# a-rtemis99/hpc_suffix_array

Measured on AMD Instinct MI355X. Metric: suffixes sorted/sec + ms/doubling-round, 1 GiB input at 1/2/4/8 MI355X, higher is better.
Workload: dtype u32

## Files before the change

### hpc_suffix_array_amd/_native.py

```python
from __future__ import annotations

import ctypes
import os
import subprocess

PKG_DIR = os.path.dirname(os.path.abspath(__file__))
LIB_PATH = os.path.join(PKG_DIR, "lib", "libsa_hip.so")
LIB_PATH = os.environ.get("SA_LIB_PATH", LIB_PATH)
CSRC = os.path.join(PKG_DIR, "csrc")

SA_MAX_ROUNDS = 64
KERNEL_KINDS = ["init", "hist_first", "hist_keys", "scan", "scatter_first", "scatter_keys",
                "heads", "heads_scan", "rerank", "seg_count", "seg_scan", "seg_write", "alphabet", "pack",
                "sort_u", "windows", "local_sort", "pivot_keys", "pivot_count", "pivot_write"]
SCHEDULE_PACKED = 0
SCHEDULE_REFERENCE = 1
ROUND1_AUTO = 0
ROUND1_LSD = 1
ROUND1_BUCKETED = 2
SA_K_COUNT = len(KERNEL_KINDS)
FIND_AUTO = 0
FIND_LANE = 1
FIND_WAVE = 2
FIND_LANE_MAX = 3584
# ... 17 lines not shown
               "sa_bwt_device", "sa_bwt", "sa_inverse_device", "sa_inverse",
               "sa_locate_device", "sa_locate",
               "sa_dist_begin", "sa_dist_cuts", "sa_dist_plan_cuts", "sa_dist_reserve", "sa_dist_release", "sa_dist_round1", "sa_dist_req_count", "sa_dist_req_fill",
               "sa_dist_answer", "sa_dist_refine",
               "sa_last_error", "sa_host_syncs", "sa_device_count", "sa_version", "sa_struct_size"]


class SAError(RuntimeError):
    """A libsa_hip entry point returned an error code."""


DEBUG_FLAGS = {"no_cmp": 0x1, "no_pk8": 0x2, "no_pad": 0x4, "pad_overflow": 0x8, "no_fast32": 0x10,
               "no_pivot": 0x20, "perm_always": 0x40, "no_xq": 0x80, "xq_overflow": 0x100,
               "no_tied": 0x200, "no_key1_round": 0x400, "no_eonly": 0x800,
               "eonly": 0x1000, "fast32_small": 0x2000, "no_round2_fused": 0x4000,
               "ls_one_wg": 0x8000}


def debug_bits(names) -> int:
    bits = 0
    for x in names or ():
        if x not in DEBUG_FLAGS:
            raise ValueError(f"unknown debug flag {x!r} (one of {sorted(DEBUG_FLAGS)})")
        bits |= DEBUG_FLAGS[x]
    return bits


class SaOpts(ctypes.Structure):
    _fields_ = [("profile", ctypes.c_int32), ("schedule", ctypes.c_int32), ("init_chars", ctypes.c_int32),
                ("radix", ctypes.c_int32), ("round1", ctypes.c_int32), ("debug", ctypes.c_uint32),
                ("span_extra", ctypes.c_int32), ("tune", ctypes.c_int32)]
# ... 13 lines not shown
        ("prefix_len", ctypes.c_uint64 * SA_MAX_ROUNDS),
        ("schedule", ctypes.c_int32),
        ("init_chars", ctypes.c_int32),
        ("sigma", ctypes.c_int32),
        ("sparse_ranks", ctypes.c_int32),
        ("round1", ctypes.c_int32),
        ("largest_window", ctypes.c_int32),
        ("model_bytes", ctypes.c_uint64),
        ("kern_ms", ctypes.c_double * SA_K_COUNT),
        ("kern_launches", ctypes.c_uint64 * SA_K_COUNT),
        ("kern_bytes", ctypes.c_uint64 * SA_K_COUNT),
        ("round1_segments", ctypes.c_int32),
        ("round1_layout", ctypes.c_int32),
        ("round_bytes", ctypes.c_uint64 * SA_MAX_ROUNDS),
        ("round1_windows", ctypes.c_int32 * 4),
    ]

    def to_dict(self) -> dict:
        r = self.rounds
        return {
            "rounds": r,
            "total_ms": self.total_ms,
            "h2d_ms": self.h2d_ms,
            "d2h_ms": self.d2h_ms,
            "round_ms": list(self.round_ms[:r]),
            "distinct": [int(x) for x in self.distinct[:r]],
            "passes": list(self.passes[:r]),
            "sorted_n": [int(x) for x in self.sorted_n[:r]],
            "prefix_len": [int(x) for x in self.prefix_len[:r]],
            "schedule": "reference" if self.schedule == SCHEDULE_REFERENCE else "packed",
            "init_chars": self.init_chars,
            "sigma": self.sigma,
            "sparse_ranks": bool(self.sparse_ranks),
            "round1": {ROUND1_LSD: "lsd", ROUND1_BUCKETED: "bucketed", 3: "pivot"}.get(self.round1, "lsd"),
            "largest_window": self.largest_window,
            "round1_segments": {0: "exact", 1: "padded", 2: "padded-overflow", 3: "striped-records",
                                4: "striped-records-overflow"}.get(self.round1_segments, "exact"),
            "round1_layout": {"compact": bool(self.round1_layout & 1), "pk8": bool(self.round1_layout & 2),
                              "xq": bool(self.round1_layout & 4), "eonly": bool(self.round1_layout & 8)},
            "reference_model_bytes": int(self.model_bytes),
            "round_bytes": [int(x) for x in self.round_bytes[:r]],
            "round1_windows": [int(x) for x in self.round1_windows],
            "kernels": {k: {"ms": self.kern_ms[i], "launches": int(self.kern_launches[i]),
                            "bytes": int(self.kern_bytes[i])} for i, k in enumerate(KERNEL_KINDS)},
        }


DIST_OK = 0
DIST_UNSUPPORTED = 1
DIST_UNBALANCED = 2


class SaDistInfo(ctypes.Structure):
    _fields_ = [("status", ctypes.c_int32), ("sigma", ctypes.c_int32), ("K", ctypes.c_int32),
                ("bucket_bits", ctypes.c_int32), ("m", ctypes.c_uint64), ("sa_off", ctypes.c_uint64),
                ("m_max", ctypes.c_uint64), ("bucket_lo", ctypes.c_uint32), ("bucket_hi", ctypes.c_uint32),
                ("round1_ok", ctypes.c_int32), ("reserved", ctypes.c_int32), ("heads", ctypes.c_uint64),
# ... 159 lines not shown
```

### hpc_suffix_array_amd/csrc/sa_build.hip

```cpp
#include <hip/hip_runtime.h>

#include <algorithm>
#include <atomic>
#include <chrono>
#include <cstdarg>
#include <cstdio>
#include <cstdlib>
#include <cstring>
#include <mutex>
#include <string>
#include <thread>
#include <vector>

#include "../../include/sa_hip.h"

#ifndef SA_ALPHA_GRID
#define SA_ALPHA_GRID 2048
#endif

#include "sa_bucket.h"
#include "sa_check.h"
#include "sa_kernels.h"
#include "sa_lcp.h"
#include "sa_limits.h"
// ... 119 lines not shown
    uint32_t* member = nullptr;
    uint32_t* hist = nullptr;
    uint32_t* totals = nullptr;
    uint32_t* counts = nullptr;
    uint32_t* words = nullptr;
    uint32_t* alpha = nullptr;
    uint16_t* code = nullptr;
    uint32_t* host_words = nullptr;
    hipEvent_t ev[sa::kEvPool + sa::kRoundEv + 1];
    int ev_ready = 0;
    sa::DistState* dist = nullptr;
    uint32_t dbg = 0;
    int32_t span_extra = 0;
    int32_t tune = 0;
    bool dna = false;
    bool samples_pending = false;
};

namespace sa {

static uint64_t pad_capacity(uint64_t n) { return n + n / 8 + (1ull << 22); }

static uint64_t pad_elems(uint64_t n) {
    const uint64_t m = align_up(std::max<uint64_t>(n, 1), 64);
    return (n >= (1ull << 26) && n <= (1ull << 31)) ? align_up(pad_capacity(n), 64) : m;
}

constexpr uint64_t kMaxRadix = 1024;
static uint64_t tile_states_bytes(uint64_t n) { return ((n + kTile - 1) / kTile + 1) * kMaxRadix * 8; }

// ... 1068 lines not shown
    *D = Dr + Dt;
    *m = mrr + T;
    *G = Gr + Gt;
    *P = 2 + Pr;
    return SA_OK;
}

static int build_packed(sa_context* c, const uint8_t* d_text, uint64_t n, uint32_t* d_sa, hipStream_t s,
                        const sa_opts* opts, sa_stats* st, Timer& tm) {
    int rc = SA_OK;
    rc = ensure_u_capacity(c, n);
    if (rc) return rc;
    tm.round_mark();
    uint32_t* h_alpha = c->host_words + 64;
    uint16_t* h_code = reinterpret_cast<uint16_t*>(c->host_words + 320);
    SA_HIP(hipMemsetAsync(c->alpha, 0, 8 * 4, s));
    tm.begin(SA_K_ALPHABET);
    {
        const uint32_t grid = (uint32_t)std::min<uint64_t>((n + kBlock * 16 - 1) / (kBlock * 16), SA_ALPHA_GRID);
        hipLaunchKernelGGL(k_alphabet, dim3(grid), dim3(kBlock), 0, s, d_text, n, c->alpha);
    }
    tm.end();
    SA_HIP(hipGetLastError());
    add_bytes(st, SA_K_ALPHABET, n);
    SA_HIP(hipMemcpyAsync(h_alpha, c->alpha, 8 * 4, hipMemcpyDeviceToHost, s));
    const uint32_t tail_n = (uint32_t)std::min<uint64_t>(n, (uint64_t)kMaxK);
    uint8_t* h_tail = reinterpret_cast<uint8_t*>(c->host_words + 2048);
    SA_HIP(hipMemcpyAsync(h_tail, d_text + (n - tail_n), tail_n, hipMemcpyDeviceToHost, s));
    SA_HIP(host_sync(s));
    uint32_t sigma = 0;
    for (int b = 0; b < 256; ++b) h_code[b] = ((h_alpha[b >> 5] >> (b & 31)) & 1u) ? (uint16_t)(++sigma) : 0;
    SA_HIP(hipMemcpyAsync(c->code, h_code, 256 * 2, hipMemcpyHostToDevice, s));
    c->dna = sigma == 4 && h_code['A'] && h_code['C'] && h_code['G'] && h_code['T'];
    uint32_t K = choose_chars(sigma, n, opts ? opts->init_chars : 0);
    const uint64_t base = (uint64_t)sigma + 1;
    const Chunking ch = plan_chunks(n);
    uint64_t* keys1 = nullptr;
    uint32_t ksh1 = 0;
    c->samples_pending = false;
    uint32_t P = 0;

    BucketPlan bp;
    const int r1 = opts ? opts->round1 : SA_ROUND1_AUTO;
    const uint32_t Kb = (opts && opts->init_chars > 0) || sigma <= 1 ? K : min_chars(sigma, n);
    bool bucketed = plan_bucketed(sigma, n, Kb, r1, c->radix, &bp, 1, (c->dbg & SA_DEBUG_NO_CMP) ? 0 : 1);
    if (bucketed && bp.bs.cmp && short_suffix_ties(h_tail, n, tail_n, h_code, sigma, bp.bs.s, bp.bs.R))
        bucketed = plan_bucketed(sigma, n, Kb, r1, c->radix, &bp, 1, 0);
    const bool force_eonly = (c->dbg & SA_DEBUG_EONLY) != 0;
    if (bucketed && bp.bs.cmp == 1 && ((sigma & (sigma - 1)) != 0 || force_eonly) && !(c->dbg & SA_DEBUG_NO_EONLY)) {
        const uint32_t hb = bp.bs.bb - kLoBits;
        BucketPlan b2;
        if ((force_eonly || !plan_pk8(bp, hb, c->dbg, true)) && plan_bucketed(sigma, n, Kb, r1, c->radix, &b2, 1, 2) &&
            (force_eonly || plan_pk8(b2, hb, c->dbg, true)) &&
            !short_suffix_ties(h_tail, n, tail_n, h_code, sigma, b2.bs.s, b2.bs.R, b2.K))
            bp = b2;
    }
    bool fused = false;
    bool r1_pivot = false;
    uint64_t D = 0, m = 0, G = 0;
    uint64_t seg1[3] = {0, 0, 0};
    int r2 = 0;
    if (bucketed) {
        bool done = false;
        rc = round1_bucketed(c, d_text, n, d_sa, bp, full_range(bp, n), s, tm, st, &done, &fused, seg1, &ksh1, true,
                             true, &r2);
        if (rc) return rc;
        bucketed = done;
        if (done) {
            keys1 = c->keys[0];
            P = 2;
            K = bp.K;
        }
    }
    if (!bucketed) {
        const uint32_t bits1 = key_bits(base, K);
        SA_TRACE("packed: sigma=%u K=%u bits=%u", sigma, K, bits1);
        uint64_t top = 1;
        for (uint32_t t = 1; t < K; ++t) top *= base;
        if (c->radix == 0) {
            rc = onesweep_prepare(c, s);
            if (rc) return rc;
        }
        tm.begin(SA_K_PACK);
        hipLaunchKernelGGL(k_pack_text, dim3(ch.chunks), dim3(kBlock), 0, s, d_text, n, (const uint16_t*)c->code, ch,
                           base, top, K, c->keys[1], c->hist, c->radix == 0 ? (bits1 + 7) / 8 : 0u, os_ghist(c));
        tm.end();
        SA_HIP(hipGetLastError());
        add_bytes(st, SA_K_PACK, 9 * n);
// ... 1258 lines not shown
```

### hpc_suffix_array_amd/csrc/sa_kernels.h

```cpp
#pragma once
#include <hip/hip_runtime.h>
#include <stdint.h>

#include "sa_search.h"

namespace sa {

constexpr int kWave = 64;
constexpr int kBlock = 256;
constexpr int kWaves = kBlock / kWave;
constexpr int kItems = 16;
constexpr int kTile = kBlock * kItems;
constexpr int kWaveTile = kWave * kItems;
constexpr int kRadix = 256;

__device__ __forceinline__ uint32_t lane_id() { return threadIdx.x & (kWave - 1); }
__device__ __forceinline__ uint32_t wave_id() { return threadIdx.x / kWave; }
__device__ __forceinline__ uint64_t lanemask_lt() { return (1ull << lane_id()) - 1ull; }

struct SrcRank {
    const uint32_t* __restrict__ rank;
    uint64_t n;
    uint64_t h;
    uint32_t w;
// ... 623 lines not shown
#pragma unroll
        for (int j = 0; j < kItems; ++j) {
            const uint64_t e = w0 + (uint64_t)j * kWave + lane_id();
            if (e < e1) {
                const uint32_t x = idx[e];
                if (x < ch.n) rank[x] = woff + (uint32_t)__popcll(m[j] & le_mask);
            }
            woff += (uint32_t)__popcll(m[j]);
        }
        run += ttot;
    }
    (void)s_tmp;
}


__global__ __launch_bounds__(kBlock) void k_alphabet(const uint8_t* __restrict__ text, uint64_t n,
                                                     uint32_t* __restrict__ present) {
    __shared__ uint32_t s_m[kBlock * 9];
    uint32_t* m = s_m + threadIdx.x * 9;
#pragma unroll
    for (int i = 0; i < 8; ++i) m[i] = 0;
    auto add = [&](uint32_t b) { atomicOr(&m[b >> 5], 1u << (b & 31u)); };
    const uint64_t stride = (uint64_t)gridDim.x * kBlock * 16;
    auto whole = [&](uint64_t i) { return i + 16 <= n && (((uintptr_t)(text + i)) & 15) == 0; };
    uint64_t i = ((uint64_t)blockIdx.x * kBlock + threadIdx.x) * 16;
    uint4 v = make_uint4(0u, 0u, 0u, 0u);
    if (i < n && whole(i)) v = *reinterpret_cast<const uint4*>(text + i);
    uint32_t step = 0;
    for (; i < n; i += stride) {
        if (step && (step & (step - 1)) == 0) {
// ... 24 lines not shown
                for (int q = 0; q < 4; ++q)
#pragma unroll
                    for (int b = 0; b < 4; ++b) bits |= 1u << ((w4[q] >> (8 * b)) & 31u);
                atomicOr(&m[(o & 0xFFu) >> 5], bits);
            } else {
#pragma unroll
                for (int q = 0; q < 4; ++q)
#pragma unroll
                    for (int b = 0; b < 4; ++b) add((w4[q] >> (8 * b)) & 0xFFu);
            }
        } else {
            for (uint64_t j = i; j < n && j < i + 16; ++j) add(text[j]);
        }
        v = vn;
    }
    __shared__ uint32_t s_or[8];
    if (threadIdx.x < 8) s_or[threadIdx.x] = 0;
    __syncthreads();
#pragma unroll
    for (int i = 0; i < 8; ++i) {
        uint32_t x = m[i];
#pragma unroll
        for (int o = 32; o >= 1; o >>= 1) x |= __shfl_xor(x, o, kWave);
        if (lane_id() == 0 && x) atomicOr(&s_or[i], x);
    }
    __syncthreads();
    if (threadIdx.x < 8) {
        const uint32_t x = s_or[threadIdx.x];
        if (x & ~__hip_atomic_load(&present[threadIdx.x], __ATOMIC_RELAXED, __HIP_MEMORY_SCOPE_AGENT))
            atomicOr(&present[threadIdx.x], x);
    }
}

__device__ __forceinline__ void hist_add_runs_valid(uint32_t (*s_h)[kRadix], uint64_t k, bool valid, uint32_t p_lo,
                                                    uint32_t p_hi, uint32_t row0) {
    const uint32_t lane = lane_id();
    const uint64_t above = lane == 63 ? 0ull : (~0ull << (lane + 1));
    for (uint32_t p = p_lo; p < p_hi; ++p) {
        const uint32_t d = valid ? ((uint32_t)(k >> (8 * p)) & 0xFFu) : 0x100u;
        const uint32_t dl = __shfl_up(d, 1, 64);
        const bool head = lane == 0 || dl != d;
        const uint64_t hm = __ballot(head) & above;
        const uint32_t next = hm ? (uint32_t)__ffsll((long long)hm) - 1u : 64u;
        if (head && valid) atomicAdd(&s_h[row0 + p][d], next - lane);
    }
}
// ... 376 lines not shown
```

### hpc_suffix_array_amd/csrc/sa_round1.h

```cpp
#pragma once

#ifndef SA_HIST_WPC
#define SA_HIST_WPC 64
#endif
#ifndef SA_REC_STRIPED
#define SA_REC_STRIPED 1
#endif
#ifndef SA_BB_EXTRA
#define SA_BB_EXTRA 0
#endif
#ifndef SA_ITEMS_A
#define SA_ITEMS_A 12
#endif
#ifndef SA_TEXT_BLOCK
#define SA_TEXT_BLOCK 512
#endif
#ifndef SA_LIST_BLOCK
#define SA_LIST_BLOCK 1024
#endif


#ifndef SA_SEG_BLOCK
#define SA_SEG_BLOCK 1024
#endif
// ... 24 lines not shown

static uint32_t text_stripes(const sa_context* c) {
    const uint32_t e = ((uint32_t)c->tune >> 8) & 0xFFu;
    const uint32_t v = e ? e : 8u;
    return v >= 8 ? 8u : v >= 4 ? 4u : v >= 2 ? 2u : 1u;
}

__global__ __launch_bounds__(kLoRadix) void k_sum_rows(const uint32_t* __restrict__ in, uint32_t rows,
                                                       uint32_t* __restrict__ out) {
    uint32_t t = 0;
    for (uint32_t r = 0; r < rows; ++r) t += in[r * kLoRadix + threadIdx.x];
    out[threadIdx.x] = t;
}
constexpr uint64_t kPadMaxN = 1ull << 31;
constexpr int kUsFlagWord = 12;

static uint32_t key1_bits(const BucketSpec& bs) {
    unsigned __int128 dmax = 1;
    for (uint32_t t = 0; t < bs.s; ++t) dmax *= bs.sigma;
    const unsigned __int128 kmax = ((dmax - 1) << bs.rb) | (((unsigned __int128)1 << bs.rb) - 1);
    uint32_t kw = 0;
    for (unsigned __int128 x = kmax + 1; x; x >>= 1) ++kw;
    return kw;
}
constexpr uint32_t kPadStartOff = kLoRadix + 1024;
constexpr uint32_t kPadDenseOff = kPadStartOff + kLoRadix + 64;

struct BucketPlan {
    BucketSpec bs{};
    uint32_t ib = 0;
// ... 256 lines not shown
    uint32_t* const cursor = stripes > 1 ? c->hist : os_ghist(c) + 5 * kRadix;
    uint32_t* const cursor_sum = stripes > 1 ? c->hist + kMaxStripes * kLoRadix : cursor;
    if (stripes > 1) SA_HIP(hipMemsetAsync(cursor, 0, (size_t)stripes * kLoRadix * 4, s));
    if (!padded) {
        tm.begin(SA_K_SCAN);
        hipLaunchKernelGGL(k_digit_base_wide, dim3(1), dim3(1024), 0, s, (const uint32_t*)g_lo, kLoRadix, os_base(c));
        tm.end();
    }
    tm.begin(SA_K_SCATTER_FIRST);
    {
        constexpr int kItemsA = SA_ITEMS_A;
        constexpr int kTextBlock = SA_TEXT_BLOCK;
        const bool pow2 = (bp.bs.sigma & (bp.bs.sigma - 1)) == 0;
        const bool dna = SA_DNA_SWAR && c->dna && bp.bs.s + bp.bs.R + kItemsA - 1 <= 32 && 2 * bp.bs.s <= 32;
        const bool ident = SA_TEXT_IDENT && bp.bs.sigma == 256 && bp.bs.s + bp.bs.R <= 8 && bp.bs.s <= 4;
        auto text_grid = [&](int block) {
            const uint64_t tile = (uint64_t)block * kItemsA;
            return (uint32_t)std::max<uint64_t>(
                1, std::min<uint64_t>((n + tile - 1) / tile, (uint64_t)c->cus * (kSpBlock / block)));
        };
#define SA_TEXT_PASS(P, PK, BLK, DNA, ID)                                                                     \
    hipLaunchKernelGGL((k_split_text<kItemsA, BLK, P, PK, DNA, ID>), dim3(text_grid(BLK)), dim3(BLK), 0, s, d_text, n, \
                       (const uint16_t*)c->code, bp.bs, (const uint32_t*)(padded ? pstart : os_base(c)),           \
                       os_tickets(c), c->keys[0], c->vals_alt, g_hi, cursor, m, blo, bhi,                          \
                       padded ? (const uint32_t*)pstart + 1 : nullptr, padded ? c->words + 11 : nullptr, hb, bp.ib, \
                       stripes)
        if (listed) {
            constexpr int kItemsL = SA_ITEMS_B, kListBlock = SA_LIST_BLOCK;
            const uint64_t tl = (uint64_t)kListBlock * kItemsL;
            const uint32_t gl = (uint32_t)std::max<uint64_t>(
                1, std::min<uint64_t>((m + tl - 1) / tl, (uint64_t)c->cus * (kSpBlock / kListBlock)));
            if (pk8)
                hipLaunchKernelGGL((k_split_list<kItemsL, kListBlock, true>), dim3(gl), dim3(kListBlock), 0, s, bp.bs,
                                   (const uint64_t*)lkeys, (const uint32_t*)lpos, m, blo, (const uint32_t*)os_base(c),
                                   os_tickets(c), c->keys[0], c->vals_alt, g_hi, cursor, hb, bp.ib,
                                   striped ? (const uint32_t*)rcur : nullptr, rcap);
            else
                hipLaunchKernelGGL((k_split_list<kItemsL, kListBlock, false>), dim3(gl), dim3(kListBlock), 0, s, bp.bs,
                                   (const uint64_t*)lkeys, (const uint32_t*)lpos, m, blo, (const uint32_t*)os_base(c),
                                   os_tickets(c), c->keys[0], c->vals_alt, g_hi, cursor, 0u, 0u,
                                   striped ? (const uint32_t*)rcur : nullptr, rcap);
        } else if (pk8 && np2) {
#define SA_TEXT_NP2(R32)                                                                                         \
    hipLaunchKernelGGL((k_split_text<kItemsA, kSpBlock, false, true, false, false, R32>), dim3(text_grid(kSpBlock)), \
                       dim3(kSpBlock), 0, s, d_text, n, (const uint16_t*)c->code, bp.bs,                           \
                       (const uint32_t*)(padded ? pstart : os_base(c)), os_tickets(c), c->keys[0], c->vals_alt, g_hi, \
                       cursor, m, blo, bhi, padded ? (const uint32_t*)pstart + 1 : nullptr,                        \
                       padded ? c->words + 11 : nullptr, hb, bp.ib, stripes)
            if (bp.bs.powR1 * (uint64_t)bp.bs.sigma <= 0xFFFFFFFFull && !(((uint32_t)c->tune >> 28) & 1u))
                SA_TEXT_NP2(true);
            else
                SA_TEXT_NP2(false);
#undef SA_TEXT_NP2
        } else if (pk8 && dna) {
            SA_TEXT_PASS(true, true, kTextBlock, true, false);
        } else if (pk8 && ident) {
            SA_TEXT_PASS(true, true, kTextBlock, false, true);
        } else if (pk8) {
            SA_TEXT_PASS(true, true, kTextBlock, false, false);
        } else if (pow2 && ident) {
            SA_TEXT_PASS(true, false, kTextBlock, false, true);
        } else if (pow2) {
            SA_TEXT_PASS(true, false, kTextBlock, false, false);
        } else if (bp.bs.powR1 * (uint64_t)bp.bs.sigma <= 0xFFFFFFFFull && !(((uint32_t)c->tune >> 28) & 1u)) {
            hipLaunchKernelGGL((k_split_text<kItemsA, kSpBlock, false, false, false, false, true>),
                               dim3(text_grid(kSpBlock)), dim3(kSpBlock), 0, s, d_text, n, (const uint16_t*)c->code,
                               bp.bs, (const uint32_t*)(padded ? pstart : os_base(c)), os_tickets(c), c->keys[0],
                               c->vals_alt, g_hi, cursor, m, blo, bhi, padded ? (const uint32_t*)pstart + 1 : nullptr,
                               padded ? c->words + 11 : nullptr, hb, bp.ib, stripes);
        } else {
            SA_TEXT_PASS(false, false, kSpBlock, false, false);
        }
#undef SA_TEXT_PASS
    }
    tm.end();
    add_bytes(st, SA_K_SCATTER_FIRST, listed ? (pk8 ? 20 : 24) * m : n + (pk8 ? 8 : 12) * m);
    tm.begin(SA_K_SCAN);
    hipLaunchKernelGGL(k_digit_base_wide, dim3(1), dim3(1024), 0, s, (const uint32_t*)g_hi, 1u << hb,
                       os_base(c) + kLoRadix);
    if (xq)
        hipLaunchKernelGGL(k_xq_dh, dim3(1), dim3(1024), 0, s, (const uint32_t*)g_hi, 1u << hb,
                           (c->dbg & SA_DEBUG_XQ_OVERFLOW) ? 1u : 0u, xq_dh);
    if (padded) {
        if (stripes > 1)
// ... 86 lines not shown
        hipLaunchKernelGGL(k_window_list, dim3(g2), dim3(kBlock), 0, s, (const uint32_t*)ws, nw, list, c->words);
    }
    tm.end();
    add_bytes(st, SA_K_WINDOWS, 8 * nw);
    SA_HIP(hipGetLastError());
    SA_HIP(hipMemcpyAsync(c->host_words, c->words, 48, hipMemcpyDeviceToHost, s));
    uint32_t* skew = list + nw;
    uint32_t* cnt_u = skew + nw;
    uint32_t* cnt_g = cnt_u + nw + 1;
    uint32_t* const rank_arr = br_.rank ? br_.rank : c->rank;
    uint32_t* const member = br_.member ? br_.member : c->member;
    SA_HIP(hipEventRecord(c->ev[kSyncEv], s));
    SA_HIP(hipMemsetAsync(cnt_u, 0, (2 * nw + 2) * 4, s));
    SA_HIP(hipMemsetAsync(member, 0, (n + 31) / 32 * 4, s));
    SA_HIP(host_sync_event(c->ev[kSyncEv]));
    if (c->host_words[4]) return set_err(SA_E_INTERNAL, "radix look-back did not complete");
    if (padded && c->host_words[11]) {
        SA_TRACE("  bucketed round 1: padded segment overflow, again with exact digit totals");
        const int rc = round1_bucketed(c, d_text, n, d_sa, bp, br_, s, tm, st, done, fused, seg, ksh, false, allow_xq,
                                       round2);
        if (st) st->round1_segments = 2;
        return rc;
    }
    if (xq && c->host_words[9]) {
        SA_TRACE("  bucketed round 1: second-pass queue overflow, again with one region");
        return round1_bucketed(c, d_text, n, d_sa, bp, br_, s, tm, st, done, fused, seg, ksh, allow_pad, false,
                               round2);
    }
    if (st) st->largest_window = (int32_t)std::min<uint32_t>(c->host_words[5], INT32_MAX);
    if (c->host_words[5] > (uint32_t)kBsCap) {
// ... 184 lines not shown
```

### hpc_suffix_array_amd/csrc/sa_split.h

```cpp
#pragma once
#include <type_traits>
#include "sa_bucket.h"
#include "sa_onesweep.h"

#ifndef SA_SEG_PROF
#define SA_SEG_PROF 0
#endif
#ifndef SA_TEXT_PROF
#define SA_TEXT_PROF 0
#endif

namespace sa {

constexpr int kSpBlock = 1024;
constexpr int kSpItems = 8;
constexpr int kSpTile = kSpBlock * kSpItems;
constexpr int kSpWaves = kSpBlock / kWave;

__device__ __forceinline__ uint32_t wave_min_u32(uint32_t x) {
#pragma unroll
    for (int o = kWave / 2; o > 0; o >>= 1) x = min(x, (uint32_t)__shfl_xor((int)x, o, kWave));
    return x;
}
__device__ __forceinline__ uint32_t wave_max_u32(uint32_t x) {
// ... 237 lines not shown
#endif
#ifndef SA_TEXT_TPT
#define SA_TEXT_TPT 4
#endif
template <int ITEMS, int BLOCK = kSpBlock, bool POW2 = false, bool PK8 = false, bool DNA = false, bool IDENT = false,
          bool R32 = false>
__global__ __launch_bounds__(BLOCK, 2048 / BLOCK) void k_split_text(const uint8_t* __restrict__ text, uint64_t n,
                                                         const uint16_t* __restrict__ code, BucketSpec b,
                                                         const uint32_t* __restrict__ digit_base,
                                                         uint32_t* __restrict__ ticket, uint64_t* __restrict__ out_keys,
                                                         uint32_t* __restrict__ out_vals,
                                                         uint32_t* __restrict__ ghist_hi, uint32_t* __restrict__ cursor,
                                                         uint64_t m, uint32_t blo, uint32_t bhi,
                                                         const uint32_t* __restrict__ seg_end = nullptr,
                                                         uint32_t* __restrict__ ovf = nullptr, uint32_t pk_hb = 0,
                                                         uint32_t pk_ib = 0, uint32_t stripes = 1) {
    constexpr bool NP2 = PK8 && !POW2;
    constexpr int RADIX = kLoRadix;
    constexpr int RWAVES = RADIX / kWave;
    constexpr int TILE = BLOCK * ITEMS;
    constexpr int kHalo = kMaxK;
    constexpr int NW = (TILE + kHalo) / 4;
    constexpr int WPT = (NW + BLOCK - 1) / BLOCK;
    static_assert(ITEMS % 4 == 0 && kHalo % 4 == 0 && TILE <= 65535, "word staging, 16-bit tile offsets");
    constexpr bool LD16 = SA_TEXT_LOAD16 != 0, SCAN1 = SA_TEXT_SCAN1 != 0, TAB1 = SA_TEXT_TAB1 != 0;
    constexpr bool EARLY = SA_TEXT_EARLY != 0;
    constexpr int NC = NW / 4;
    static_assert(!LD16 || (NW % 4 == 0 && NC <= BLOCK && WPT <= 4), "one 16-byte chunk per lane");
    static_assert(!SCAN1 || RADIX == 4 * kWave, "wave 0 scans four digits per lane");
    __shared__ uint64_t s_keys[TILE];
    __shared__ uint16_t s_idx[TILE];
    __shared__ __attribute__((aligned(16))) uint32_t s_dcw[(DNA && LD16) ? 4 : NW + 8];
    __shared__ uint32_t s_pkw[DNA ? (NW + 3) / 4 + 4 : 1];
    __shared__ uint8_t s_map[256];
    __shared__ __attribute__((aligned(16))) uint32_t s_cnt[RADIX];
    __shared__ __attribute__((aligned(8))) uint16_t s_start[RADIX];
    constexpr uint32_t kTabSkip = ~0u;
    __shared__ uint32_t s_gofs[RADIX];
    __shared__ uint32_t s_tmp[RWAVES];
    __shared__ uint32_t s_tile[2];
    __shared__ uint32_t s_kept;
    __shared__ uint32_t s_hhi[1024];
    __shared__ uint32_t s_gend[RADIX];
    const uint8_t* s_dc = reinterpret_cast<const uint8_t*>(s_dcw);
    const uint32_t bspan = bhi - blo;
    bool over = false;

    const uint32_t wave = wave_id(), lane = lane_id();
    const uint32_t dg = threadIdx.x;
    const uint64_t tiles = (n + TILE - 1) / TILE;
    const uint32_t K = b.s + b.R;
    const uint32_t stripe = blockIdx.x % stripes;
    uint32_t sbase = 0;
    for (uint32_t i = dg; i < 1024u; i += BLOCK) s_hhi[i] = 0;
    if (seg_end && dg < (uint32_t)RADIX) {
        const uint32_t lo = digit_base[dg], hi = seg_end[dg], sc = (hi - lo) / stripes;
        sbase = lo + stripe * sc;
        s_gend[dg] = stripe + 1 == stripes ? hi : sbase + sc;
    }
    cursor += stripe * RADIX;
    if (dg < 256u) {
        const uint32_t cv = code[dg];
        s_map[dg] = (uint8_t)(cv ? cv - 1u : 0u);
    }
    if (dg < (uint32_t)RADIX) s_cnt[dg] = 0;
    constexpr uint32_t TPT = SA_TEXT_TPT;
    static_assert(TPT >= 1 && (TPT & (TPT - 1)) == 0, "tiles per ticket: a power of two");
    const uint32_t tpt = tiles >= 128ull * gridDim.x ? TPT : tiles >= 32ull * gridDim.x && TPT > 1 ? TPT / 2 : 1u;
    uint32_t tk_tile = 0, tk_left = 0;
    auto next_tile = [&]() -> uint32_t {
        if constexpr (TPT == 1) {
            return atomicAdd(ticket, 1u);
        } else {
            if (tk_left == 0) {
                tk_tile = atomicAdd(ticket, 1u) * tpt;
                tk_left = tpt;
            }
            --tk_left;
// ... 38 lines not shown
    if (t < tiles) load(t);
    uint32_t par = 0;
    const uint32_t t_int = n >= (uint64_t)TILE + K ? (uint32_t)((n - TILE - K) / TILE + 1) : 0u;
    const uint32_t t_last = (uint32_t)(tiles - 1);
#if SA_TEXT_PROF
    uint64_t pacc[5] = {0, 0, 0, 0, 0}, plast = clock64();
#define TEXT_STAMP(k)                               \
    if (dg == 0) {                                  \
        const uint64_t now_ = clock64();            \
        pacc[k] += now_ - plast;                    \
        plast = now_;                               \
    }
#else
#define TEXT_STAMP(k)
#endif
    auto stage = [&](uint64_t tt) {
        const uint64_t tb = tt * TILE;
        const bool whole = (uint32_t)tt < t_whole;
        if constexpr (LD16) {
            if (dg < (uint32_t)NC) {
                uint32_t o[4];
#pragma unroll
                for (int i = 0; i < 4; ++i) {
                    o[i] = 0;
                    if (whole) {
                        if constexpr (DNA)
                            o[i] = ((raw[i] >> 1) ^ (raw[i] >> 2)) & 0x03030303u;
                        else if constexpr (IDENT)
                            o[i] = raw[i];
                        else
                            o[i] = (uint32_t)s_map[raw[i] & 0xFFu] | ((uint32_t)s_map[(raw[i] >> 8) & 0xFFu] << 8) |
                                   ((uint32_t)s_map[(raw[i] >> 16) & 0xFFu] << 16) |
                                   ((uint32_t)s_map[raw[i] >> 24] << 24);
                    } else {
#pragma unroll
                        for (int q = 0; q < 4; ++q) {
                            const uint64_t pos = tb + 16ull * dg + 4ull * i + q;
                            o[i] |= (pos < n ? (uint32_t)s_map[(raw[i] >> (8 * q)) & 0xFFu] : 0u) << (8 * q);
                        }
                    }
                }
                if constexpr (DNA) {
                    uint32_t pw = 0;
#pragma unroll
                    for (int i = 0; i < 4; ++i)
                        pw |= ((((o[i] & 3u) << 6) | ((o[i] >> 4) & 0x30u) | ((o[i] >> 14) & 0xCu) | (o[i] >> 24)) & 0xFFu)
                              << (8 * i);
                    s_pkw[dg] = pw;
                } else {
                    *reinterpret_cast<uint4*>(&s_dcw[4 * dg]) = make_uint4(o[0], o[1], o[2], o[3]);
                }
            }
        } else {
#pragma unroll
        for (int i = 0; i < WPT; ++i) {
            const uint32_t w = dg + i * BLOCK;
            if (w < (uint32_t)NW) {
                uint32_t o = 0;
                if (whole) {
                    if constexpr (DNA)
                        o = ((raw[i] >> 1) ^ (raw[i] >> 2)) & 0x03030303u;
                    else if constexpr (IDENT)
                        o = raw[i];
                    else
                        o = (uint32_t)s_map[raw[i] & 0xFFu] | ((uint32_t)s_map[(raw[i] >> 8) & 0xFFu] << 8) |
                            ((uint32_t)s_map[(raw[i] >> 16) & 0xFFu] << 16) | ((uint32_t)s_map[raw[i] >> 24] << 24);
                } else {
#pragma unroll
                    for (int q = 0; q < 4; ++q) {
                        const uint64_t pos = tb + 4ull * w + q;
                        o |= (pos < n ? (uint32_t)s_map[(raw[i] >> (8 * q)) & 0xFFu] : 0u) << (8 * q);
                    }
                }
                s_dcw[w] = o;
                if constexpr (DNA)
                    reinterpret_cast<uint8_t*>(s_pkw)[w] =
                        (uint8_t)(((o & 3u) << 6) | ((o >> 4) & 0x30u) | ((o >> 14) & 0xCu) | (o >> 24));
            }
        }
        }
    };
    if constexpr (EARLY) {
        if (t < tiles) stage(t);
        __syncthreads();
    }
    while (t < tiles) {
        const uint64_t tb = t * TILE;
        const uint32_t valid = (uint32_t)t < t_last ? (uint32_t)TILE : (uint32_t)(n - tb);
// ... 210 lines not shown
                        if constexpr (!PK8) out_vals[g] = (uint32_t)(tb + s_idx[q]);
                    } else {
                        over = true;
                    }
                }
            }
        }
        __syncthreads();
        TEXT_STAMP(4)
        t = tn;
        par ^= 1u;
    }
    for (uint32_t i = dg; i < 1024u; i += BLOCK)
        if (s_hhi[i]) atomicAdd(&ghist_hi[i], s_hhi[i]);
    if (over && ovf) atomicOr(ovf, 1u);
#if SA_TEXT_PROF
    if (dg == 0 && (blockIdx.x == 0 || blockIdx.x == gridDim.x / 2))
        printf("k_split_text wg %u clk: stage %llu keys %llu claims %llu scatter %llu write %llu\n", blockIdx.x,
               (unsigned long long)pacc[0], (unsigned long long)pacc[1], (unsigned long long)pacc[2],
               (unsigned long long)pacc[3], (unsigned long long)pacc[4]);
#endif
#undef TEXT_STAMP
}

template <int ITEMS, int BLOCK = kSpBlock, bool PK8 = false>
__global__ __launch_bounds__(BLOCK, 2048 / BLOCK) void k_split_list(BucketSpec b, const uint64_t* __restrict__ lkeys,
                                                         const uint32_t* __restrict__ lpos, uint64_t m, uint32_t blo,
                                                         const uint32_t* __restrict__ digit_base,
                                                         uint32_t* __restrict__ ticket, uint64_t* __restrict__ out_keys,
                                                         uint32_t* __restrict__ out_vals,
// ... 495 lines not shown
```

### include/sa_hip.h

```cpp
#ifndef SA_HIP_H
#define SA_HIP_H

#include <stdint.h>

#ifdef __cplusplus
extern "C" {
#endif

#define SA_OK 0
#define SA_E_INVALID (-1)
#define SA_E_NOMEM (-2)
#define SA_E_HIP (-3)
#define SA_E_INTERNAL (-4)

#define SA_MAX_ROUNDS 64

enum sa_kernel_kind {
    SA_K_INIT = 0,
    SA_K_HIST_FIRST = 1,
    SA_K_HIST_KEYS = 2,
    SA_K_SCAN = 3,
    SA_K_SCATTER_FIRST = 4,
    SA_K_SCATTER_KEYS = 5,
    SA_K_HEADS = 6,
// ... 25 lines not shown
#define SA_DEBUG_NO_PK8 0x2u
#define SA_DEBUG_NO_PAD 0x4u
#define SA_DEBUG_PAD_OVERFLOW 0x8u
#define SA_DEBUG_NO_FAST32 0x10u
#define SA_DEBUG_NO_PIVOT 0x20u
#define SA_DEBUG_PERM_ALWAYS 0x40u
#define SA_DEBUG_NO_XQ 0x80u
#define SA_DEBUG_XQ_OVERFLOW 0x100u
#define SA_DEBUG_NO_KEY1_ROUND 0x400u
#define SA_DEBUG_NO_TIED 0x200u
#define SA_DEBUG_NO_EONLY 0x800u
#define SA_DEBUG_EONLY 0x1000u
#define SA_DEBUG_FAST32_SMALL 0x2000u
#define SA_DEBUG_NO_ROUND2_FUSED 0x4000u
#define SA_DEBUG_LS_ONE_WG 0x8000u

typedef struct {
    int32_t profile;
    int32_t schedule;
    int32_t init_chars;
    int32_t radix;
    int32_t round1;
    uint32_t debug;
    int32_t span_extra;
    int32_t tune;
} sa_opts;

typedef struct {
    int32_t rounds;
    int32_t n_kinds;
// ... 6 lines not shown
    uint64_t prefix_len[SA_MAX_ROUNDS];
    int32_t schedule;
    int32_t init_chars;
    int32_t sigma;
    int32_t sparse_ranks;
    int32_t round1;
    int32_t largest_window;
    uint64_t model_bytes;
    double kern_ms[SA_K_COUNT];
    uint64_t kern_launches[SA_K_COUNT];
    uint64_t kern_bytes[SA_K_COUNT];
    int32_t round1_segments;
    int32_t round1_layout;
    uint64_t round_bytes[SA_MAX_ROUNDS];
    int32_t round1_windows[4];
} sa_stats;

typedef struct sa_context sa_context;

int sa_context_create(int device, uint64_t max_n, sa_context** out);
int sa_context_set_debug(sa_context* ctx, const sa_opts* opts);
void sa_context_destroy(sa_context* ctx);
uint64_t sa_workspace_bytes(uint64_t max_n);

int sa_build_device(sa_context* ctx, const uint8_t* d_text, uint64_t n, uint32_t* d_sa,
                    void* stream, const sa_opts* opts, sa_stats* stats);

int sa_build_ex(const uint8_t* text, uint64_t n, void* sa_out, int sa_width,
                const sa_opts* opts, sa_stats* stats);

// ... 130 lines not shown
```

Measured before the change: 109.1 billion.

## Sample the alphabet speculatively and verify it during the first bucketed pass

Replaces the full-text alphabet scan with a kernel that reads roughly one 4 KiB block in 64, plus the tail. The first bucketed round-1 pass then checks each mapped byte against the sampled alphabet and flags any byte outside it. If such a byte appears, the whole round is redone with the exact alphabet. This removes a full read of the 1 GiB input before round 1, at the cost of extra per-byte checks in the split kernel and a full rerun when the sample misses a symbol.

```diff
diff --git a/hpc_suffix_array_amd/_native.py b/hpc_suffix_array_amd/_native.py
--- a/hpc_suffix_array_amd/_native.py
+++ b/hpc_suffix_array_amd/_native.py
@@ -55,7 +55,7 @@
                "no_pivot": 0x20, "perm_always": 0x40, "no_xq": 0x80, "xq_overflow": 0x100,
                "no_tied": 0x200, "no_key1_round": 0x400, "no_eonly": 0x800,
                "eonly": 0x1000, "fast32_small": 0x2000, "no_round2_fused": 0x4000,
-               "ls_one_wg": 0x8000}
+               "ls_one_wg": 0x8000, "no_alpha_sample": 0x10000, "alpha_sample_small": 0x20000}
 
 
 def debug_bits(names) -> int:
@@ -99,6 +99,7 @@
         ("round1_layout", ctypes.c_int32),
         ("round_bytes", ctypes.c_uint64 * SA_MAX_ROUNDS),
         ("round1_windows", ctypes.c_int32 * 4),
+        ("alphabet", ctypes.c_int32),
     ]
 
     def to_dict(self) -> dict:
@@ -126,6 +127,7 @@
             "reference_model_bytes": int(self.model_bytes),
             "round_bytes": [int(x) for x in self.round_bytes[:r]],
             "round1_windows": [int(x) for x in self.round1_windows],
+            "alphabet": {0: "exact", 1: "sampled", 2: "refuted"}.get(self.alphabet, "exact"),
             "kernels": {k: {"ms": self.kern_ms[i], "launches": int(self.kern_launches[i]),
                             "bytes": int(self.kern_bytes[i])} for i, k in enumerate(KERNEL_KINDS)},
         }
diff --git a/hpc_suffix_array_amd/csrc/sa_alpha.h b/hpc_suffix_array_amd/csrc/sa_alpha.h
--- /dev/null
+++ b/hpc_suffix_array_amd/csrc/sa_alpha.h
@@ -0,0 +1,60 @@
+#pragma once
+#include <stdint.h>
+
+#if defined(__HIPCC__) || defined(__HIP__)
+#define SA_HD __host__ __device__ __forceinline__
+#else
+#define SA_HD inline
+#endif
+
+namespace sa {
+
+constexpr uint32_t kAlphaBlock = 4096;
+constexpr uint32_t kAlphaEvery = 64;
+
+SA_HD uint64_t alpha_text_blocks(uint64_t n) { return (n + kAlphaBlock - 1) / kAlphaBlock; }
+
+SA_HD uint64_t alpha_sample_blocks(uint64_t n, bool first4k) {
+    const uint64_t nb = alpha_text_blocks(n);
+    if (first4k || nb <= 1) return nb ? 1 : 0;
+    const uint64_t ns = n / ((uint64_t)kAlphaBlock * kAlphaEvery);
+    return ns < 2 ? 2 : ns;
+}
+
+SA_HD uint64_t alpha_block(uint64_t j, uint64_t nb, uint64_t ns) {
+    return ns <= 1 ? 0 : (uint64_t)(((unsigned __int128)j * (nb - 1)) / (ns - 1));
+}
+
+SA_HD uint64_t alpha_sample_bytes(uint64_t n, bool first4k) {
+    const uint64_t nb = alpha_text_blocks(n), ns = alpha_sample_blocks(n, first4k);
+    if (ns == 0) return 0;
+    const uint64_t last = alpha_block(ns - 1, nb, ns);
+    const uint64_t last_len = last + 1 == nb ? n - last * kAlphaBlock : kAlphaBlock;
+    return (ns - 1) * kAlphaBlock + last_len;
+}
+
+SA_HD uint32_t dna_digits(uint32_t w) { return ((w >> 1) ^ (w >> 2)) & 0x03030303u; }
+
+SA_HD uint32_t select_bytes(uint32_t tab, uint32_t sel) {
+#if defined(__HIP_DEVICE_COMPILE__)
+    return __builtin_amdgcn_perm(0u, tab, sel);
+#else
+    uint32_t r = 0;
+    for (int i = 0; i < 4; ++i) r |= ((tab >> (8 * ((sel >> (8 * i)) & 3u))) & 0xFFu) << (8 * i);
+    return r;
+#endif
+}
+
+SA_HD uint32_t dna_foreign(uint32_t w, uint32_t dig) { return w ^ select_bytes(0x54474341u , dig); }
+
+constexpr uint32_t kAlphaAbsent = 0xFFu;
+
+SA_HD uint32_t alpha_map_entry(uint32_t code ) {
+    return code ? code - 1u : kAlphaAbsent;
+}
+
+SA_HD uint32_t absent_bytes(uint32_t m) { return ((m & 0x7F7F7F7Fu) + 0x01010101u) & m & 0x80808080u; }
+
+SA_HD uint32_t absent_to_zero(uint32_t m, uint32_t a) { return m & ~(a | (a - (a >> 7))); }
+
+}
diff --git a/hpc_suffix_array_amd/csrc/sa_build.hip b/hpc_suffix_array_amd/csrc/sa_build.hip
--- a/hpc_suffix_array_amd/csrc/sa_build.hip
+++ b/hpc_suffix_array_amd/csrc/sa_build.hip
@@ -157,6 +157,8 @@
     int32_t span_extra = 0;
     int32_t tune = 0;
     bool dna = false;
+    bool alpha_prove = false;
+    bool alpha_refuted = false;
     bool samples_pending = false;
 };
 
@@ -1255,64 +1257,105 @@
     tm.round_mark();
     uint32_t* h_alpha = c->host_words + 64;
     uint16_t* h_code = reinterpret_cast<uint16_t*>(c->host_words + 320);
-    SA_HIP(hipMemsetAsync(c->alpha, 0, 8 * 4, s));
-    tm.begin(SA_K_ALPHABET);
-    {
-        const uint32_t grid = (uint32_t)std::min<uint64_t>((n + kBlock * 16 - 1) / (kBlock * 16), SA_ALPHA_GRID);
-        hipLaunchKernelGGL(k_alphabet, dim3(grid), dim3(kBlock), 0, s, d_text, n, c->alpha);
-    }
-    tm.end();
-    SA_HIP(hipGetLastError());
-    add_bytes(st, SA_K_ALPHABET, n);
-    SA_HIP(hipMemcpyAsync(h_alpha, c->alpha, 8 * 4, hipMemcpyDeviceToHost, s));
     const uint32_t tail_n = (uint32_t)std::min<uint64_t>(n, (uint64_t)kMaxK);
     uint8_t* h_tail = reinterpret_cast<uint8_t*>(c->host_words + 2048);
-    SA_HIP(hipMemcpyAsync(h_tail, d_text + (n - tail_n), tail_n, hipMemcpyDeviceToHost, s));
-    SA_HIP(host_sync(s));
-    uint32_t sigma = 0;
-    for (int b = 0; b < 256; ++b) h_code[b] = ((h_alpha[b >> 5] >> (b & 31)) & 1u) ? (uint16_t)(++sigma) : 0;
-    SA_HIP(hipMemcpyAsync(c->code, h_code, 256 * 2, hipMemcpyHostToDevice, s));
-    c->dna = sigma == 4 && h_code['A'] && h_code['C'] && h_code['G'] && h_code['T'];
-    uint32_t K = choose_chars(sigma, n, opts ? opts->init_chars : 0);
-    const uint64_t base = (uint64_t)sigma + 1;
-    const Chunking ch = plan_chunks(n);
+    uint32_t sigma = 0, K = 0, Kb = 0;
+    BucketPlan bp;
+    const int r1 = opts ? opts->round1 : SA_ROUND1_AUTO;
+    bool bucketed = false;
+    auto plan_round1 = [&](bool sampled, bool* complete) -> int {
+        SA_HIP(hipMemsetAsync(c->alpha, 0, 8 * 4, s));
+        tm.begin(SA_K_ALPHABET);
+        if (sampled) {
+            const bool first4k = (c->dbg & SA_DEBUG_ALPHA_SAMPLE_SMALL) != 0;
+            const uint64_t nb = alpha_text_blocks(n), ns = alpha_sample_blocks(n, first4k);
+            hipLaunchKernelGGL(k_alphabet_sample, dim3((uint32_t)std::min<uint64_t>(ns, 2ull * (uint32_t)c->cus)),
+                               dim3(kBlock), 0, s, d_text, n, nb, ns, c->alpha);
+            add_bytes(st, SA_K_ALPHABET, alpha_sample_bytes(n, first4k));
+        } else {
+            const uint32_t grid = (uint32_t)std::min<uint64_t>((n + kBlock * 16 - 1) / (kBlock * 16), SA_ALPHA_GRID);
+            hipLaunchKernelGGL(k_alphabet, dim3(grid), dim3(kBlock), 0, s, d_text, n, c->alpha);
+            add_bytes(st, SA_K_ALPHABET, n);
+        }
+        tm.end();
+        SA_HIP(hipGetLastError());
+        SA_HIP(hipMemcpyAsync(h_alpha, c->alpha, 8 * 4, hipMemcpyDeviceToHost, s));
+        SA_HIP(hipMemcpyAsync(h_tail, d_text + (n - tail_n), tail_n, hipMemcpyDeviceToHost, s));
+        SA_HIP(host_sync(s));
+        *complete = true;
+        for (uint32_t t = 0; t < tail_n; ++t) {
+            const uint32_t x = h_tail[t];
+            if (!((h_alpha[x >> 5] >> (x & 31)) & 1u)) *complete = false;
+            h_alpha[x >> 5] |= 1u << (x & 31);
+        }
+        sigma = 0;
+        for (int b = 0; b < 256; ++b) h_code[b] = ((h_alpha[b >> 5] >> (b & 31)) & 1u) ? (uint16_t)(++sigma) : 0;
+        SA_HIP(hipMemcpyAsync(c->code, h_code, 256 * 2, hipMemcpyHostToDevice, s));
+        c->dna = sigma == 4 && h_code['A'] && h_code['C'] && h_code['G'] && h_code['T'];
+        K = choose_chars(sigma, n, opts ? opts->init_chars : 0);
+        Kb = (opts && opts->init_chars > 0) || sigma <= 1 ? K : min_chars(sigma, n);
+        bucketed = plan_bucketed(sigma, n, Kb, r1, c->radix, &bp, 1, (c->dbg & SA_DEBUG_NO_CMP) ? 0 : 1);
+        if (bucketed && bp.bs.cmp && short_suffix_ties(h_tail, n, tail_n, h_code, sigma, bp.bs.s, bp.bs.R))
+            bucketed = plan_bucketed(sigma, n, Kb, r1, c->radix, &bp, 1, 0);
+        const bool force_eonly = (c->dbg & SA_DEBUG_EONLY) != 0;
+        if (bucketed && bp.bs.cmp == 1 && ((sigma & (sigma - 1)) != 0 || force_eonly) &&
+            !(c->dbg & SA_DEBUG_NO_EONLY)) {
+            const uint32_t hb = bp.bs.bb - kLoBits;
+            BucketPlan b2;
+            if ((force_eonly || !plan_pk8(bp, hb, c->dbg, true)) && plan_bucketed(sigma, n, Kb, r1, c->radix, &b2, 1, 2) &&
+                (force_eonly || plan_pk8(b2, hb, c->dbg, true)) &&
+                !short_suffix_ties(h_tail, n, tail_n, h_code, sigma, b2.bs.s, b2.bs.R, b2.K))
+                bp = b2;
+        }
+        return SA_OK;
+    };
+    bool sampled = !(c->dbg & SA_DEBUG_NO_ALPHA_SAMPLE) &&
+                   (n >= kPadMinN || (c->dbg & SA_DEBUG_ALPHA_SAMPLE_SMALL)) && c->radix == 0 && r1 != SA_ROUND1_LSD;
+    bool refuted = false;
     uint64_t* keys1 = nullptr;
     uint32_t ksh1 = 0;
-    c->samples_pending = false;
     uint32_t P = 0;
-
-    BucketPlan bp;
-    const int r1 = opts ? opts->round1 : SA_ROUND1_AUTO;
-    const uint32_t Kb = (opts && opts->init_chars > 0) || sigma <= 1 ? K : min_chars(sigma, n);
-    bool bucketed = plan_bucketed(sigma, n, Kb, r1, c->radix, &bp, 1, (c->dbg & SA_DEBUG_NO_CMP) ? 0 : 1);
-    if (bucketed && bp.bs.cmp && short_suffix_ties(h_tail, n, tail_n, h_code, sigma, bp.bs.s, bp.bs.R))
-        bucketed = plan_bucketed(sigma, n, Kb, r1, c->radix, &bp, 1, 0);
-    const bool force_eonly = (c->dbg & SA_DEBUG_EONLY) != 0;
-    if (bucketed && bp.bs.cmp == 1 && ((sigma & (sigma - 1)) != 0 || force_eonly) && !(c->dbg & SA_DEBUG_NO_EONLY)) {
-        const uint32_t hb = bp.bs.bb - kLoBits;
-        BucketPlan b2;
-        if ((force_eonly || !plan_pk8(bp, hb, c->dbg, true)) && plan_bucketed(sigma, n, Kb, r1, c->radix, &b2, 1, 2) &&
-            (force_eonly || plan_pk8(b2, hb, c->dbg, true)) &&
-            !short_suffix_ties(h_tail, n, tail_n, h_code, sigma, b2.bs.s, b2.bs.R, b2.K))
-            bp = b2;
-    }
     bool fused = false;
     bool r1_pivot = false;
     uint64_t D = 0, m = 0, G = 0;
     uint64_t seg1[3] = {0, 0, 0};
     int r2 = 0;
-    if (bucketed) {
+    for (;;) {
+        bool complete = true;
+        rc = plan_round1(sampled, &complete);
+        if (rc) return rc;
+        if (sampled && !(bucketed && complete)) {
+            SA_TRACE("packed: sampled alphabet (sigma=%u) not kept: %s", sigma,
+                     complete ? "round 1 is not bucketed" : "the tail holds another symbol");
+            sampled = false;
+            continue;
+        }
+        c->samples_pending = false;
+        if (!bucketed) break;
         bool done = false;
+        c->alpha_prove = sampled && sigma < 256;
+        c->alpha_refuted = false;
         rc = round1_bucketed(c, d_text, n, d_sa, bp, full_range(bp, n), s, tm, st, &done, &fused, seg1, &ksh1, true,
                              true, &r2);
+        c->alpha_prove = false;
         if (rc) return rc;
+        if (c->alpha_refuted) {
+            SA_TRACE("packed: the first pass met a symbol outside the sampled alphabet, again with the exact one");
+            sampled = false;
+            refuted = true;
+            continue;
+        }
         bucketed = done;
         if (done) {
             keys1 = c->keys[0];
             P = 2;
             K = bp.K;
         }
-    }
+        break;
+    }
+    if (st) st->alphabet = refuted ? SA_ALPHABET_REFUTED : sampled ? SA_ALPHABET_SAMPLED : SA_ALPHABET_EXACT;
+    const uint64_t base = (uint64_t)sigma + 1;
+    const Chunking ch = plan_chunks(n);
     if (!bucketed) {
         const uint32_t bits1 = key_bits(base, K);
         SA_TRACE("packed: sigma=%u K=%u bits=%u", sigma, K, bits1);
diff --git a/hpc_suffix_array_amd/csrc/sa_kernels.h b/hpc_suffix_array_amd/csrc/sa_kernels.h
--- a/hpc_suffix_array_amd/csrc/sa_kernels.h
+++ b/hpc_suffix_array_amd/csrc/sa_kernels.h
@@ -2,6 +2,7 @@
 #include <hip/hip_runtime.h>
 #include <stdint.h>
 
+#include "sa_alpha.h"
 #include "sa_search.h"
 
 namespace sa {
@@ -661,6 +662,25 @@
 }
 
 
+__device__ __forceinline__ void alphabet_reduce(const uint32_t* m, uint32_t* __restrict__ present) {
+    __shared__ uint32_t s_or[8];
+    if (threadIdx.x < 8) s_or[threadIdx.x] = 0;
+    __syncthreads();
+#pragma unroll
+    for (int i = 0; i < 8; ++i) {
+        uint32_t x = m[i];
+#pragma unroll
+        for (int o = 32; o >= 1; o >>= 1) x |= __shfl_xor(x, o, kWave);
+        if (lane_id() == 0 && x) atomicOr(&s_or[i], x);
+    }
+    __syncthreads();
+    if (threadIdx.x < 8) {
+        const uint32_t x = s_or[threadIdx.x];
+        if (x & ~__hip_atomic_load(&present[threadIdx.x], __ATOMIC_RELAXED, __HIP_MEMORY_SCOPE_AGENT))
+            atomicOr(&present[threadIdx.x], x);
+    }
+}
+
 __global__ __launch_bounds__(kBlock) void k_alphabet(const uint8_t* __restrict__ text, uint64_t n,
                                                      uint32_t* __restrict__ present) {
     __shared__ uint32_t s_m[kBlock * 9];
@@ -715,22 +735,43 @@
         }
         v = vn;
     }
-    __shared__ uint32_t s_or[8];
-    if (threadIdx.x < 8) s_or[threadIdx.x] = 0;
-    __syncthreads();
-#pragma unroll
-    for (int i = 0; i < 8; ++i) {
-        uint32_t x = m[i];
-#pragma unroll
-        for (int o = 32; o >= 1; o >>= 1) x |= __shfl_xor(x, o, kWave);
-        if (lane_id() == 0 && x) atomicOr(&s_or[i], x);
-    }
-    __syncthreads();
-    if (threadIdx.x < 8) {
-        const uint32_t x = s_or[threadIdx.x];
-        if (x & ~__hip_atomic_load(&present[threadIdx.x], __ATOMIC_RELAXED, __HIP_MEMORY_SCOPE_AGENT))
-            atomicOr(&present[threadIdx.x], x);
-    }
+    alphabet_reduce(m, present);
+}
+
+__global__ __launch_bounds__(kBlock) void k_alphabet_sample(const uint8_t* __restrict__ text, uint64_t n, uint64_t nb,
+                                                            uint64_t ns, uint32_t* __restrict__ present) {
+    static_assert(kBlock * 16 == (int)kAlphaBlock, "one 16-byte chunk per lane and block");
+    __shared__ uint32_t s_m[kBlock * 9];
+    uint32_t* m = s_m + threadIdx.x * 9;
+#pragma unroll
+    for (int i = 0; i < 8; ++i) m[i] = 0;
+    auto add = [&](uint32_t b) { atomicOr(&m[b >> 5], 1u << (b & 31u)); };
+    const bool al16 = (((uintptr_t)text) & 15) == 0;
+    constexpr int kFlight = 4;
+    for (uint64_t j0 = blockIdx.x; j0 < ns; j0 += (uint64_t)kFlight * gridDim.x) {
+        uint4 v[kFlight];
+        uint64_t at[kFlight];
+#pragma unroll
+        for (int q = 0; q < kFlight; ++q) {
+            const uint64_t j = j0 + (uint64_t)q * gridDim.x;
+            at[q] = j < ns ? alpha_block(j, nb, ns) * kAlphaBlock + threadIdx.x * 16u : n;
+            v[q] = make_uint4(0u, 0u, 0u, 0u);
+            if (al16 && at[q] + 16 <= n) v[q] = *reinterpret_cast<const uint4*>(text + at[q]);
+        }
+#pragma unroll
+        for (int q = 0; q < kFlight; ++q) {
+            if (al16 && at[q] + 16 <= n) {
+                const uint32_t w4[4] = {v[q].x, v[q].y, v[q].z, v[q].w};
+#pragma unroll
+                for (int w = 0; w < 4; ++w)
+#pragma unroll
+                    for (int b = 0; b < 4; ++b) add((w4[w] >> (8 * b)) & 0xFFu);
+            } else {
+                for (uint64_t k = at[q]; k < n && k < at[q] + 16; ++k) add(text[k]);
+            }
+        }
+    }
+    alphabet_reduce(m, present);
 }
 
 __device__ __forceinline__ void hist_add_runs_valid(uint32_t (*s_h)[kRadix], uint64_t k, bool valid, uint32_t p_lo,
diff --git a/hpc_suffix_array_amd/csrc/sa_round1.h b/hpc_suffix_array_amd/csrc/sa_round1.h
--- a/hpc_suffix_array_amd/csrc/sa_round1.h
+++ b/hpc_suffix_array_amd/csrc/sa_round1.h
@@ -62,6 +62,7 @@
 }
 constexpr uint64_t kPadMaxN = 1ull << 31;
 constexpr int kUsFlagWord = 12;
+constexpr int kAlphaBadWord = 8;
 
 static uint32_t key1_bits(const BucketSpec& bs) {
     unsigned __int128 dmax = 1;
@@ -348,6 +349,7 @@
         const bool pow2 = (bp.bs.sigma & (bp.bs.sigma - 1)) == 0;
         const bool dna = SA_DNA_SWAR && c->dna && bp.bs.s + bp.bs.R + kItemsA - 1 <= 32 && 2 * bp.bs.s <= 32;
         const bool ident = SA_TEXT_IDENT && bp.bs.sigma == 256 && bp.bs.s + bp.bs.R <= 8 && bp.bs.s <= 4;
+        uint32_t* const alpha_bad = c->alpha_prove && !listed ? c->words + kAlphaBadWord : nullptr;
         auto text_grid = [&](int block) {
             const uint64_t tile = (uint64_t)block * kItemsA;
             return (uint32_t)std::max<uint64_t>(
@@ -358,7 +360,7 @@
                        (const uint16_t*)c->code, bp.bs, (const uint32_t*)(padded ? pstart : os_base(c)),           \
                        os_tickets(c), c->keys[0], c->vals_alt, g_hi, cursor, m, blo, bhi,                          \
                        padded ? (const uint32_t*)pstart + 1 : nullptr, padded ? c->words + 11 : nullptr, hb, bp.ib, \
-                       stripes)
+                       stripes, alpha_bad)
         if (listed) {
             constexpr int kItemsL = SA_ITEMS_B, kListBlock = SA_LIST_BLOCK;
             const uint64_t tl = (uint64_t)kListBlock * kItemsL;
@@ -380,7 +382,7 @@
                        dim3(kSpBlock), 0, s, d_text, n, (const uint16_t*)c->code, bp.bs,                           \
                        (const uint32_t*)(padded ? pstart : os_base(c)), os_tickets(c), c->keys[0], c->vals_alt, g_hi, \
                        cursor, m, blo, bhi, padded ? (const uint32_t*)pstart + 1 : nullptr,                        \
-                       padded ? c->words + 11 : nullptr, hb, bp.ib, stripes)
+                       padded ? c->words + 11 : nullptr, hb, bp.ib, stripes, alpha_bad)
             if (bp.bs.powR1 * (uint64_t)bp.bs.sigma <= 0xFFFFFFFFull && !(((uint32_t)c->tune >> 28) & 1u))
                 SA_TEXT_NP2(true);
             else
@@ -401,7 +403,7 @@
                                dim3(text_grid(kSpBlock)), dim3(kSpBlock), 0, s, d_text, n, (const uint16_t*)c->code,
                                bp.bs, (const uint32_t*)(padded ? pstart : os_base(c)), os_tickets(c), c->keys[0],
                                c->vals_alt, g_hi, cursor, m, blo, bhi, padded ? (const uint32_t*)pstart + 1 : nullptr,
-                               padded ? c->words + 11 : nullptr, hb, bp.ib, stripes);
+                               padded ? c->words + 11 : nullptr, hb, bp.ib, stripes, alpha_bad);
         } else {
             SA_TEXT_PASS(false, false, kSpBlock, false, false);
         }
@@ -518,6 +520,10 @@
     SA_HIP(hipMemsetAsync(cnt_u, 0, (2 * nw + 2) * 4, s));
     SA_HIP(hipMemsetAsync(member, 0, (n + 31) / 32 * 4, s));
     SA_HIP(host_sync_event(c->ev[kSyncEv]));
+    if (c->alpha_prove && c->host_words[kAlphaBadWord]) {
+        c->alpha_refuted = true;
+        return SA_OK;
+    }
     if (c->host_words[4]) return set_err(SA_E_INTERNAL, "radix look-back did not complete");
     if (padded && c->host_words[11]) {
         SA_TRACE("  bucketed round 1: padded segment overflow, again with exact digit totals");
diff --git a/hpc_suffix_array_amd/csrc/sa_split.h b/hpc_suffix_array_amd/csrc/sa_split.h
--- a/hpc_suffix_array_amd/csrc/sa_split.h
+++ b/hpc_suffix_array_amd/csrc/sa_split.h
@@ -1,5 +1,6 @@
 #pragma once
 #include <type_traits>
+#include "sa_alpha.h"
 #include "sa_bucket.h"
 #include "sa_onesweep.h"
 
@@ -275,7 +276,8 @@
                                                          uint64_t m, uint32_t blo, uint32_t bhi,
                                                          const uint32_t* __restrict__ seg_end = nullptr,
                                                          uint32_t* __restrict__ ovf = nullptr, uint32_t pk_hb = 0,
-                                                         uint32_t pk_ib = 0, uint32_t stripes = 1) {
+                                                         uint32_t pk_ib = 0, uint32_t stripes = 1,
+                                                         uint32_t* __restrict__ alpha_bad = nullptr) {
     constexpr bool NP2 = PK8 && !POW2;
     constexpr int RADIX = kLoRadix;
     constexpr int RWAVES = RADIX / kWave;
@@ -306,6 +308,8 @@
     const uint8_t* s_dc = reinterpret_cast<const uint8_t*>(s_dcw);
     const uint32_t bspan = bhi - blo;
     bool over = false;
+    const bool prove = !IDENT && alpha_bad != nullptr;
+    bool foreign = false;
 
     const uint32_t wave = wave_id(), lane = lane_id();
     const uint32_t dg = threadIdx.x;
@@ -322,7 +326,7 @@
     cursor += stripe * RADIX;
     if (dg < 256u) {
         const uint32_t cv = code[dg];
-        s_map[dg] = (uint8_t)(cv ? cv - 1u : 0u);
+        s_map[dg] = (uint8_t)(prove ? alpha_map_entry(cv) : cv ? cv - 1u : 0u);
     }
     if (dg < (uint32_t)RADIX) s_cnt[dg] = 0;
     constexpr uint32_t TPT = SA_TEXT_TPT;
@@ -391,32 +395,52 @@
 #else
 #define TEXT_STAMP(k)
 #endif
+    auto map4 = [&](uint32_t w, uint32_t& bad) -> uint32_t {
+        if constexpr (DNA) {
+            const uint32_t o = dna_digits(w);
+            bad |= dna_foreign(w, o);
+            return o;
+        } else if constexpr (IDENT) {
+            return w;
+        } else {
+            uint32_t o = (uint32_t)s_map[w & 0xFFu] | ((uint32_t)s_map[(w >> 8) & 0xFFu] << 8) |
+                         ((uint32_t)s_map[(w >> 16) & 0xFFu] << 16) | ((uint32_t)s_map[w >> 24] << 24);
+            if (prove) {
+                const uint32_t a = absent_bytes(o);
+                bad |= a;
+                o = absent_to_zero(o, a);
+            }
+            return o;
+        }
+    };
+    auto map1 = [&](uint32_t x, uint32_t& bad) -> uint32_t {
+        uint32_t v = s_map[x];
+        if (prove) {
+            bad |= v == kAlphaAbsent ? 1u : 0u;
+            v = v == kAlphaAbsent ? 0u : v;
+        }
+        return v;
+    };
     auto stage = [&](uint64_t tt) {
         const uint64_t tb = tt * TILE;
         const bool whole = (uint32_t)tt < t_whole;
         if constexpr (LD16) {
             if (dg < (uint32_t)NC) {
-                uint32_t o[4];
+                uint32_t o[4], bad = 0;
 #pragma unroll
                 for (int i = 0; i < 4; ++i) {
                     o[i] = 0;
                     if (whole) {
-                        if constexpr (DNA)
-                            o[i] = ((raw[i] >> 1) ^ (raw[i] >> 2)) & 0x03030303u;
-                        else if constexpr (IDENT)
-                            o[i] = raw[i];
-                        else
-                            o[i] = (uint32_t)s_map[raw[i] & 0xFFu] | ((uint32_t)s_map[(raw[i] >> 8) & 0xFFu] << 8) |
-                                   ((uint32_t)s_map[(raw[i] >> 16) & 0xFFu] << 16) |
-                                   ((uint32_t)s_map[raw[i] >> 24] << 24);
+                        o[i] = map4(raw[i], bad);
                     } else {
 #pragma unroll
                         for (int q = 0; q < 4; ++q) {
                             const uint64_t pos = tb + 16ull * dg + 4ull * i + q;
-                            o[i] |= (pos < n ? (uint32_t)s_map[(raw[i] >> (8 * q)) & 0xFFu] : 0u) << (8 * q);
+                            o[i] |= (pos < n ? map1((raw[i] >> (8 * q)) & 0xFFu, bad) : 0u) << (8 * q);
                         }
                     }
                 }
+                foreign |= bad != 0u;
                 if constexpr (DNA) {
                     uint32_t pw = 0;
 #pragma unroll
@@ -433,22 +457,17 @@
         for (int i = 0; i < WPT; ++i) {
             const uint32_t w = dg + i * BLOCK;
             if (w < (uint32_t)NW) {
-                uint32_t o = 0;
+                uint32_t o = 0, bad = 0;
                 if (whole) {
-                    if constexpr (DNA)
-                        o = ((raw[i] >> 1) ^ (raw[i] >> 2)) & 0x03030303u;
-                    else if constexpr (IDENT)
-                        o = raw[i];
-                    else
-                        o = (uint32_t)s_map[raw[i] & 0xFFu] | ((uint32_t)s_map[(raw[i] >> 8) & 0xFFu] << 8) |
-                            ((uint32_t)s_map[(raw[i] >> 16) & 0xFFu] << 16) | ((uint32_t)s_map[raw[i] >> 24] << 24);
+                    o = map4(raw[i], bad);
                 } else {
 #pragma unroll
                     for (int q = 0; q < 4; ++q) {
                         const uint64_t pos = tb + 4ull * w + q;
-                        o |= (pos < n ? (uint32_t)s_map[(raw[i] >> (8 * q)) & 0xFFu] : 0u) << (8 * q);
+                        o |= (pos < n ? map1((raw[i] >> (8 * q)) & 0xFFu, bad) : 0u) << (8 * q);
                     }
                 }
+                foreign |= bad != 0u;
                 s_dcw[w] = o;
                 if constexpr (DNA)
                     reinterpret_cast<uint8_t*>(s_pkw)[w] =
@@ -689,6 +708,7 @@
     for (uint32_t i = dg; i < 1024u; i += BLOCK)
         if (s_hhi[i]) atomicAdd(&ghist_hi[i], s_hhi[i]);
     if (over && ovf) atomicOr(ovf, 1u);
+    if (foreign && alpha_bad) atomicOr(alpha_bad, 1u);
 #if SA_TEXT_PROF
     if (dg == 0 && (blockIdx.x == 0 || blockIdx.x == gridDim.x / 2))
         printf("k_split_text wg %u clk: stage %llu keys %llu claims %llu scatter %llu write %llu\n", blockIdx.x,
diff --git a/include/sa_hip.h b/include/sa_hip.h
--- a/include/sa_hip.h
+++ b/include/sa_hip.h
@@ -63,6 +63,12 @@
 #define SA_DEBUG_FAST32_SMALL 0x2000u
 #define SA_DEBUG_NO_ROUND2_FUSED 0x4000u
 #define SA_DEBUG_LS_ONE_WG 0x8000u
+#define SA_DEBUG_NO_ALPHA_SAMPLE 0x10000u
+#define SA_DEBUG_ALPHA_SAMPLE_SMALL 0x20000u
+
+#define SA_ALPHABET_EXACT 0
+#define SA_ALPHABET_SAMPLED 1
+#define SA_ALPHABET_REFUTED 2
 
 typedef struct {
     int32_t profile;
@@ -99,6 +105,7 @@
     int32_t round1_layout;
     uint64_t round_bytes[SA_MAX_ROUNDS];
     int32_t round1_windows[4];
+    int32_t alphabet;
 } sa_stats;
 
 typedef struct sa_context sa_context;
```

Measured after the change: 110.8 billion (median of 6 runs). +1.5%, better.
